# leejaehot/GaussianGrasper

Hardware: AMD Instinct MI355X
Metric: rendered views/sec (fwd+bwd) at 1M Gaussians, 1600x1200, 32-ch feature (higher is better)
Workload: dtype f32; 1 GPU; BASELINE config 4 per-GPU share: 1000000 Gaussians, 1600x1200, SH deg 4 rgb + 32-ch feature + depth + normal images per view (nerfstudio plugin route: the timed callable is FusedGaussianSplattingModel.get_outputs(camera) of gaussiangrasper_amd.plugin (the class train.sh loads, on stub.py's stand-ins for nerfstudio's base model and Cameras) — one fused rasterize operator per view), fwd+bwd, 8 views; route=plugin, deterministic_backward=False, python_gc=gc.freeze() after the warm-up (bench.freeze_gc), view_pipeline=backward of view k beside forward of view k + 1 on two streams, num_gaussians=1000000, feature_dim=32, n_visible=992125, parallelism=view-parallel x1, replicated Gaussians, grad_allreduce_bytes=472000000, grad_allreduce=per parameter, overlapped with the last view's backward

## Files before the change

gaussiangrasper_amd/csrc/binning.hip:

```cpp
#include "scan.h"

__device__ __forceinline__ int64_t dev_count(int64_t n, const int64_t *__restrict__ n_dev) {
    if (n_dev) {
        const int64_t d = *n_dev;
        if (d < n) n = d;
    }
    return n;
}

#define RS_THREADS 256
#define RS_WAVES (RS_THREADS / GG_WAVE)
#ifndef GG_RS_BIG
#define GG_RS_BIG 16
#endif
static inline int rs_items(int64_t n) { return n >= (int64_t)4096 * 1024 ? GG_RS_BIG : 4; }

__global__ __launch_bounds__(256) void count_kernel(int N, const int32_t *__restrict__ nth,
                                                    unsigned long long *__restrict__ out) {
    __shared__ unsigned long long part[4];
    unsigned long long acc = 0;
    for (int i = blockIdx.x * blockDim.x + threadIdx.x; i < N; i += gridDim.x * blockDim.x)
        acc += (unsigned long long)(uint32_t)nth[i];
    for (int off = 32; off > 0; off >>= 1) acc += __shfl_down(acc, off, 64);
    if ((threadIdx.x & 63) == 0) part[threadIdx.x >> 6] = acc;
    __syncthreads();
    if (threadIdx.x == 0) atomicAdd(out, part[0] + part[1] + part[2] + part[3]);
}

extern "C" size_t gg_count_workspace(int num_points) {
    (void)num_points;
    return 0;
}
extern "C" int gg_count_intersects(int N, const int32_t *num_tiles_hit, int64_t *out, void *ws,
                                   size_t ws_bytes, gg_stream_t stream) {
    (void)ws;
    (void)ws_bytes;
    GG_REQUIRE(N >= 0, "num_points < 0");
    GG_REQUIRE(out != nullptr, "null output");
    hipStream_t s = (hipStream_t)stream;
    if (gg_fill_async(out, 0, sizeof(int64_t), s) != hipSuccess) {
        gg_set_error("gg_count_intersects: memset failed");
        return GG_ERR_LAUNCH;
    }
    if (N == 0) return GG_OK;
    GG_REQUIRE(num_tiles_hit != nullptr, "null pointer");
    int blocks = min((N + 255) / 256, 128);
    gg_prof_begin(GG_K_COUNT, s);
    hipLaunchKernelGGL(count_kernel, dim3(blocks), dim3(256), 0, s, N, num_tiles_hit,
                       (unsigned long long *)out);
    gg_prof_end(GG_K_COUNT, s);
    GG_CHECK_LAUNCH();
    return GG_OK;
}

struct DepthSrc {
    const float *depths;
    const int32_t *radii;
};
__device__ __forceinline__ uint32_t depth_key(const DepthSrc d, int64_t idx) {
    return (d.radii[idx] > 0) ? __builtin_bit_cast(uint32_t, d.depths[idx]) : 0xFFFFFFFFu;
}

template <int RS_ITEMS>
__global__ __launch_bounds__(RS_THREADS) void radix_hist_kernel(
    int64_t n, const int64_t *__restrict__ n_dev, const uint32_t *__restrict__ keys, int shift,
    uint32_t mask, int nblocks, uint32_t *__restrict__ G, DepthSrc dsrc) {
    constexpr int RS_TILE = RS_THREADS * RS_ITEMS;
    __shared__ uint32_t hist[256];
    n = dev_count(n, n_dev);
    hist[threadIdx.x] = 0;
    __syncthreads();
    int64_t base = (int64_t)blockIdx.x * RS_TILE;
#pragma unroll 4
    for (int it = 0; it < RS_ITEMS; ++it) {
        int64_t idx = base + (int64_t)it * RS_THREADS + threadIdx.x;
        if (idx < n) atomicAdd(&hist[((dsrc.depths ? depth_key(dsrc, idx) : keys[idx]) >> shift) & mask], 1u);
    }
    __syncthreads();
    G[(size_t)threadIdx.x * nblocks + blockIdx.x] = hist[threadIdx.x];
}

__global__ __launch_bounds__(256) void radix_colscan_kernel(int nblocks, uint32_t *__restrict__ G,
                                                            uint32_t *__restrict__ totals) {
    __shared__ uint32_t wsum[4];
    __shared__ uint32_t carry_s;
    uint32_t *row = G + (size_t)blockIdx.x * nblocks;
    const int lane = threadIdx.x & 63, wave = threadIdx.x >> 6;
    if (threadIdx.x == 0) carry_s = 0;
    __syncthreads();
    for (int start = 0; start < nblocks; start += 256) {
        int i = start + threadIdx.x;
        uint32_t v = (i < nblocks) ? row[i] : 0u;
        uint32_t incl = v;
        for (int off = 1; off < 64; off <<= 1) {
            uint32_t t = __shfl_up(incl, off, 64);
            if (lane >= off) incl += t;
        }
        if (lane == 63) wsum[wave] = incl;
        __syncthreads();
        uint32_t wpre = 0;
        for (int w = 0; w < wave; ++w) wpre += wsum[w];
        uint32_t carry = carry_s;
        if (i < nblocks) row[i] = carry + wpre + incl - v;
        __syncthreads();
        if (threadIdx.x == 255) carry_s = carry + wpre + incl;
        __syncthreads();
    }
    if (threadIdx.x == 0) totals[blockIdx.x] = carry_s;
}

template <int RS_ITEMS>
__global__ __launch_bounds__(RS_THREADS) void radix_scatter_kernel(
    int64_t n, const int64_t *__restrict__ n_dev, const uint32_t *__restrict__ keys_in,
    const uint32_t *__restrict__ vals_in, uint32_t *__restrict__ keys_out,
    uint32_t *__restrict__ vals_out, int shift, uint32_t mask, int nblocks,
    const uint32_t *__restrict__ G, const uint32_t *__restrict__ totals, DepthSrc dsrc) {
    constexpr int RS_TILE = RS_THREADS * RS_ITEMS;
    n = dev_count(n, n_dev);
    const int nbits = 32 - __builtin_clz(mask | 1u);
    __shared__ uint32_t whist[RS_WAVES][256];
    __shared__ uint32_t digit_base[256];
    __shared__ uint32_t wsum[4];
    const int tid = threadIdx.x, lane = tid & 63, wave = tid >> 6;
    {
        uint32_t v = totals[tid];
        uint32_t incl = v;
        for (int off = 1; off < 64; off <<= 1) {
            uint32_t t = __shfl_up(incl, off, 64);
            if (lane >= off) incl += t;
        }
        if (lane == 63) wsum[wave] = incl;
        for (int w = 0; w < RS_WAVES; ++w) whist[w][tid] = 0;
        __syncthreads();
        uint32_t wpre = 0;
        for (int w = 0; w < wave; ++w) wpre += wsum[w];
        digit_base[tid] = wpre + incl - v + G[(size_t)tid * nblocks + blockIdx.x];
    }
    __syncthreads();

    const int64_t wbase = (int64_t)blockIdx.x * RS_TILE + (int64_t)wave * (GG_WAVE * RS_ITEMS);
    uint32_t key[RS_ITEMS], val[RS_ITEMS], rank[RS_ITEMS];
    const uint64_t lt_mask = (lane == 0) ? 0ull : (~0ull >> (64 - lane));
#pragma unroll
    for (int it = 0; it < RS_ITEMS; ++it) {
        int64_t idx = wbase + (int64_t)it * GG_WAVE + lane;
        bool valid = idx < n;
        key[it] = valid ? (dsrc.depths ? depth_key(dsrc, idx) : keys_in[idx]) : 0u;
        val[it] = valid ? (dsrc.depths ? (uint32_t)idx : vals_in[idx]) : 0u;
    }
#pragma unroll
    for (int it = 0; it < RS_ITEMS; ++it) {
        int64_t idx = wbase + (int64_t)it * GG_WAVE + lane;
        bool valid = idx < n;
        uint32_t d = (key[it] >> shift) & mask;
        uint64_t peers = __ballot(valid);
#pragma unroll
        for (int b = 0; b < 8; ++b) {
            if (b < nbits) {
                bool bit = (d >> b) & 1u;
                uint64_t m = __ballot(bit);
                peers &= bit ? m : ~m;
            }
        }
        uint32_t cnt = (uint32_t)__popcll(peers);
        uint32_t before = (uint32_t)__popcll(peers & lt_mask);
        uint32_t old = 0u;
        if (valid && before == 0) old = atomicAdd(&whist[wave][d], cnt);
        old = __shfl(old, (int)__builtin_ctzll(peers | (1ull << 63)), 64);
        rank[it] = old + before;
    }
    __syncthreads();
    __shared__ uint32_t lstart[256];
    __shared__ uint32_t skey[RS_TILE], sval[RS_TILE];
    {
        uint32_t run = 0;
        for (int w = 0; w < RS_WAVES; ++w) {
            uint32_t c = whist[w][tid];
            whist[w][tid] = run;
            run += c;
        }
        uint32_t incl = run;
        for (int off = 1; off < 64; off <<= 1) {
            uint32_t u = __shfl_up(incl, off, 64);
            if (lane >= off) incl += u;
        }
        if (lane == 63) wsum[wave] = incl;
        __syncthreads();
        uint32_t wpre = 0;
        for (int w = 0; w < wave; ++w) wpre += wsum[w];
        lstart[tid] = wpre + incl - run;
    }
    __syncthreads();
#pragma unroll
    for (int it = 0; it < RS_ITEMS; ++it) {
        int64_t idx = wbase + (int64_t)it * GG_WAVE + lane;
        if (idx < n) {
            uint32_t d = (key[it] >> shift) & mask;
            uint32_t lp = lstart[d] + whist[wave][d] + rank[it];
            skey[lp] = key[it];
            sval[lp] = val[it];
        }
    }
    __syncthreads();
    const int64_t left = n - (int64_t)blockIdx.x * RS_TILE;
    const int count = (int)(left < RS_TILE ? left : RS_TILE);
    for (int jj = tid; jj < count; jj += RS_THREADS) {
        const uint32_t k = skey[jj];
        const uint32_t d = (k >> shift) & mask;
        const uint32_t dst = digit_base[d] + ((uint32_t)jj - lstart[d]);
        keys_out[dst] = k;
        vals_out[dst] = sval[jj];
    }
}


typedef unsigned long long u64;
#define DB_BLOCKS 64
#define DB_THREADS 1024
#define DB_CAP 512
// ... 451 lines not shown
#pragma unroll
            for (int r = 0; r < DB_ITEMS; ++r) gid[r] = (c0 + 64 * r + lane < n) ? (uint32_t)pairs[s0 + c0 + 64 * r + lane] : 0u;
        }
#pragma unroll
        for (int r = 0; r < DB_ITEMS; ++r) {
            const int p = c0 + 64 * r + lane;
            if (c0 + 64 * r < n) {
                const bool valid = p < n;
                const uint32_t g = min(gid[r], (uint32_t)(N - 1));
                uint32_t c = cntv[r], bx = boxv[r];
                if (!carried) {
                    c = 0u;
                    bx = 1u << 20;
                    if (valid) db_box(geom, dsrc, (int)g, c, bx);
                }
                if (!valid) c = 0u;
                uint32_t incl = c;
#pragma unroll
                for (int off = 1; off < 64; off <<= 1) {
                    const uint32_t u = __shfl_up(incl, off, 64);
                    if (lane >= off) incl += u;
                }
                if (valid) {
                    order[s0 + p] = g;
                    einfo[s0 + p] = make_uint4(carry + incl - c, (uint32_t)b, bx, c);
                }
                carry += __shfl(incl, 63, 64);
            }
        }
    }
    if (lane == 0) bucket_sum[b] = carry;
}

__global__ __launch_bounds__(256) void emit_kernel(int N, const uint32_t *__restrict__ order,
                                                   const uint4 *__restrict__ einfo,
                                                   const uint32_t *__restrict__ bucket_base,
                                                   const uint32_t *__restrict__ visible, int tiles_x,
                                                   int64_t I, const int64_t *__restrict__ I_dev,
                                                   uint32_t *__restrict__ tkeys,
                                                   uint32_t *__restrict__ tvals) {
    __shared__ uint32_t s_rel[4][64];
    I = dev_count(I, I_dev);
    __shared__ int4 s_box[4][64];
    const int lane = threadIdx.x & 63, wave = threadIdx.x >> 6;
    const int r = blockIdx.x * blockDim.x + threadIdx.x;
    uint32_t g = 0, cnt = 0, off = 0;
    int x0 = 0, y0 = 0, bw = 1;
    if (r < N && (uint32_t)r < *visible) {
        g = min(order[r], (uint32_t)(N - 1));
        const uint4 e = einfo[r];
        off = e.x + bucket_base[e.y];
        x0 = (int)(e.z & 1023u);
        y0 = (int)((e.z >> 10) & 1023u);
        bw = max(1, (int)(e.z >> 20));
        cnt = e.w;
    }
    uint32_t incl = cnt;
    for (int d = 1; d < 64; d <<= 1) {
        uint32_t u = __shfl_up(incl, d, 64);
        if (lane >= d) incl += u;
    }
    const uint32_t total = __shfl(incl, 63, 64);
    const uint32_t base = __shfl(off, 0, 64);
    s_rel[wave][lane] = incl - cnt;
    s_box[wave][lane] = make_int4(x0, y0, bw, (int)g);
    __builtin_amdgcn_wave_barrier();
    const uint32_t *rel = s_rel[wave];
    for (uint32_t j = lane; j < total; j += 64) {
        int lo = 0;
#pragma unroll
        for (int step = 32; step > 0; step >>= 1)
            if (rel[lo + step] <= j) lo += step;
        const int4 b = s_box[wave][lo];
        const uint32_t k = j - rel[lo];
        const uint32_t row = k / (uint32_t)b.z;
        const int64_t cur = (int64_t)base + j;
        if (cur < I) {
            tkeys[cur] = (uint32_t)((b.y + (int)row) * tiles_x + b.x + (int)(k - row * (uint32_t)b.z));
            tvals[cur] = (uint32_t)b.w;
        }
    }
}

__global__ __launch_bounds__(256) void tile_bins_kernel(int64_t I, const int64_t *__restrict__ I_dev,
                                                        const uint32_t *__restrict__ tkeys_sorted,
                                                        uint32_t num_tiles,
                                                        int32_t *__restrict__ tile_bins,
                                                        int32_t *__restrict__ tile_out) {
    I = dev_count(I, I_dev);
    int64_t i = (int64_t)blockIdx.x * blockDim.x + threadIdx.x;
    if (i >= I) return;
    uint32_t cur = tkeys_sorted[i];
    if (tile_out) tile_out[i] = (int32_t)cur;
    const bool cur_ok = cur < num_tiles;
    if (i == 0 && cur_ok) tile_bins[2 * cur] = 0;
    if (i == I - 1 && cur_ok) tile_bins[2 * cur + 1] = (int32_t)I;
    if (i > 0) {
        uint32_t prev = tkeys_sorted[i - 1];
        if (prev != cur) {
            if (prev < num_tiles) tile_bins[2 * prev + 1] = (int32_t)i;
            if (cur_ok) tile_bins[2 * cur] = (int32_t)i;
        }
    }
}

static int radix_nblocks(int64_t n) {
    const int64_t tile = (int64_t)RS_THREADS * rs_items(n);
    return (int)((n + tile - 1) / tile);
}

struct BinWs {
    uint32_t *order;
    uint4 *einfo;
    uint32_t *G;
    uint32_t *totals;
    uint32_t *tkeyA, *tkeyB, *tvalTmp;
    uint4 *recs;
    u64 *pairs;
    uint32_t *dbG;
    uint32_t *dbStart;
    uint32_t *dbBase;
    uint32_t *dbmm;
    size_t bytes;
};
static BinWs bin_ws_layout(void *ws, int N, int64_t I) {
    BinWs w;
    size_t off = 0;
    auto take = [&](size_t nbytes) {
        char *p = ws ? (char *)ws + off : nullptr;
        off += gg_align_up(nbytes, 256);
        return (uint32_t *)p;
    };
    size_t n = (size_t)(N > 0 ? N : 1), i = (size_t)(I > 0 ? I : 1);
    w.order = take(4 * n);
    w.einfo = (uint4 *)take(16 * n);
    int nb = max(radix_nblocks(N), radix_nblocks(I));
    w.G = take(4 * 256 * (size_t)(nb + 1));
    w.totals = take(4 * 256);
    w.tkeyA = take(4 * i);
    w.tkeyB = take(4 * i);
    w.tvalTmp = take(4 * i);
    const size_t nbk = (size_t)db_buckets(N);
    w.recs = (uint4 *)take(16 * n);
    w.pairs = (u64 *)take(8 * n);
    w.dbG = take(4 * DB_BLOCKS * (nbk + 1));
    w.dbStart = take(4 * (nbk + 2));
    w.dbBase = take(4 * (nbk + 1));
    w.dbmm = take(4 * 2 * 256);
    w.bytes = off;
    return w;
}
extern "C" size_t gg_bin_sort_workspace(int num_points, int64_t num_intersects) {
    return bin_ws_layout(nullptr, num_points, num_intersects).bytes;
}

static void radix_pass(int64_t n, const int64_t *n_dev, const uint32_t *kin, const uint32_t *vin,
                       uint32_t *kout, uint32_t *vout, int shift, uint32_t mask, BinWs &w, hipStream_t s,
                       DepthSrc dsrc = DepthSrc{nullptr, nullptr}) {
    int nb = radix_nblocks(n);
    if (rs_items(n) != 4)
        hipLaunchKernelGGL(radix_hist_kernel<GG_RS_BIG>, dim3(nb), dim3(RS_THREADS), 0, s, n, n_dev, kin, shift,
                           mask, nb, w.G, dsrc);
    else
        hipLaunchKernelGGL(radix_hist_kernel<4>, dim3(nb), dim3(RS_THREADS), 0, s, n, n_dev, kin, shift,
                           mask, nb, w.G, dsrc);
    hipLaunchKernelGGL(radix_colscan_kernel, dim3(256), dim3(256), 0, s, nb, w.G, w.totals);
    if (rs_items(n) != 4)
        hipLaunchKernelGGL(radix_scatter_kernel<GG_RS_BIG>, dim3(nb), dim3(RS_THREADS), 0, s, n, n_dev, kin, vin,
                           kout, vout, shift, mask, nb, w.G, w.totals, dsrc);
    else
        hipLaunchKernelGGL(radix_scatter_kernel<4>, dim3(nb), dim3(RS_THREADS), 0, s, n, n_dev, kin, vin,
                           kout, vout, shift, mask, nb, w.G, w.totals, dsrc);
}

static int bin_sort_impl(int N, int64_t I, const int64_t *I_dev, const float *xys, const float *depths,
                         const int32_t *radii, const int32_t *num_tiles_hit, int tiles_x, int tiles_y,
                         int32_t *gaussian_ids_sorted, int32_t *tile_bins, int32_t *isect_tile_sorted,
                         void *ws, size_t ws_bytes, gg_stream_t stream, const uint32_t *range_lo = nullptr,
                         const uint32_t *range_hi = nullptr, int range_parts = 0) {
    GG_REQUIRE(N >= 0 && I >= 0, "negative size");
    GG_REQUIRE(tiles_x > 0 && tiles_y > 0, "empty tile grid");
    GG_REQUIRE(tiles_x <= DB_BOX_MAX && tiles_y <= DB_BOX_MAX, "tile grid beyond 1023 x 1023 (images beyond 16 368 pixels a side)");
    GG_REQUIRE(I < (int64_t)1 << 31, "num_intersects must fit int32 (tile_bins are int32)");
    GG_REQUIRE(tile_bins != nullptr, "null tile_bins");
    hipStream_t s = (hipStream_t)stream;
    const int T = tiles_x * tiles_y;
    if (N == 0 || I == 0) {
        if (gg_fill_async(tile_bins, 0, sizeof(int32_t) * 2 * (size_t)T, s) != hipSuccess) {
            gg_set_error("gg_bin_sort: memset failed");
            return GG_ERR_LAUNCH;
        }
        return GG_OK;
    }
    GG_REQUIRE(xys && depths && radii && num_tiles_hit && gaussian_ids_sorted, "null pointer");
    BinWs w = bin_ws_layout(ws, N, I);
    if (ws == nullptr || ws_bytes < w.bytes) {
        gg_set_error("gg_bin_sort: workspace too small (%zu < %zu)", ws_bytes, w.bytes);
        return GG_ERR_WORKSPACE;
    }
    gg_prof_begin(GG_K_BIN_SORT, s);
    const int nbk = db_buckets(N);
    const DepthSrc dsrc{depths, radii};
    const size_t walk_lds = sizeof(uint32_t) * ((size_t)nbk + 1 + 2);
    if (walk_lds > 64 * 1024) {
        (void)hipFuncSetAttribute((const void *)db_walk_kernel<false>, hipFuncAttributeMaxDynamicSharedMemorySize, (int)walk_lds);
        (void)hipFuncSetAttribute((const void *)db_walk_kernel<true>, hipFuncAttributeMaxDynamicSharedMemorySize, (int)walk_lds);
    }
    uint32_t *order = w.order;
    DbParts mm{w.dbmm, w.dbmm + 256, 256};
    if (range_lo && range_hi && range_parts > 0)
        mm = DbParts{range_lo, range_hi, range_parts};
    else
        hipLaunchKernelGGL(db_range_kernel, dim3(256), dim3(256), 0, s, N, dsrc, w.dbmm);
    const DbGeom geom{xys, tiles_x, tiles_y};
    hipLaunchKernelGGL(db_walk_kernel<false>, dim3(DB_BLOCKS), dim3(DB_THREADS), walk_lds, s, N, nbk, dsrc, geom, mm,
                       w.dbG, (const uint32_t *)nullptr, (uint4 *)nullptr, tile_bins, 2 * T);
    hipLaunchKernelGGL(db_prefix_kernel, dim3((nbk + 1 + 255) / 256), dim3(256), 0, s, nbk, w.dbG, w.dbStart);
    hipLaunchKernelGGL(db_scan_kernel, dim3(1), dim3(1024), 0, s, nbk, w.dbStart);
    hipLaunchKernelGGL(db_walk_kernel<true>, dim3(DB_BLOCKS), dim3(DB_THREADS), walk_lds, s, N, nbk, dsrc, geom, mm,
                       w.dbG, (const uint32_t *)w.dbStart, w.recs, (int32_t *)nullptr, 0);
    hipLaunchKernelGGL(db_sort_kernel, dim3((nbk + DB_WPB - 1) / DB_WPB), dim3(64 * DB_WPB), 0, s, N, nbk,
                       (const uint32_t *)w.dbStart, (const uint4 *)w.recs, w.pairs, dsrc, geom, order, w.einfo, w.dbBase);
    hipLaunchKernelGGL(db_scan_kernel, dim3(1), dim3(1024), 0, s, nbk, w.dbBase);
    int tile_bits = 1;
    while ((1 << tile_bits) < T) ++tile_bits;
    int passes = (tile_bits + 7) / 8;
    uint32_t *out_vals = (uint32_t *)gaussian_ids_sorted;
    uint32_t *kcur = w.tkeyA, *kalt = w.tkeyB;
    uint32_t *vcur = (passes % 2 == 0) ? out_vals : w.tvalTmp;
    uint32_t *valt = (passes % 2 == 0) ? w.tvalTmp : out_vals;
    if (!I_dev) {
        (void)gg_fill_async(kcur, 0xFF, sizeof(uint32_t) * (size_t)I, s);
        (void)gg_fill_async(vcur, 0, sizeof(uint32_t) * (size_t)I, s);
    }
    hipLaunchKernelGGL(emit_kernel, dim3((N + 255) / 256), dim3(256), 0, s, N, (const uint32_t *)order,
                       (const uint4 *)w.einfo, (const uint32_t *)w.dbBase, (const uint32_t *)(w.dbStart + nbk), tiles_x, I,
                       I_dev, kcur, vcur);
    const int per_pass = (tile_bits + passes - 1) / passes;
    for (int pass = 0; pass < passes; ++pass) {
        int bits = min(per_pass, tile_bits - per_pass * pass);
        radix_pass(I, I_dev, kcur, vcur, kalt, valt, per_pass * pass, (1u << bits) - 1u, w, s);
        uint32_t *t = kcur; kcur = kalt; kalt = t;
        t = vcur; vcur = valt; valt = t;
    }
    hipLaunchKernelGGL(tile_bins_kernel, dim3((unsigned)((I + 255) / 256)), dim3(256), 0, s, I, I_dev, kcur,
                       (uint32_t)T, tile_bins, isect_tile_sorted);
    gg_prof_end(GG_K_BIN_SORT, s);
    GG_CHECK_LAUNCH();
    return GG_OK;
}

extern "C" int gg_bin_sort_status(int N, int64_t I, const void *ws, size_t ws_bytes, gg_stream_t stream) {
    GG_REQUIRE(N >= 0 && I >= 0, "negative size");
    (void)ws;
    (void)ws_bytes;
    if (hipStreamSynchronize((hipStream_t)stream) != hipSuccess) {
        gg_set_error("gg_bin_sort_status: stream synchronisation failed");
        return GG_ERR_LAUNCH;
    }
    return GG_OK;
}

extern "C" int gg_bin_sort(int N, int64_t I, const float *xys, const float *depths,
                           const int32_t *radii, const int32_t *num_tiles_hit, int tiles_x,
                           int tiles_y, int32_t *gaussian_ids_sorted, int32_t *tile_bins,
                           int32_t *isect_tile_sorted, void *ws, size_t ws_bytes,
                           gg_stream_t stream) {
    return bin_sort_impl(N, I, nullptr, xys, depths, radii, num_tiles_hit, tiles_x, tiles_y,
                         gaussian_ids_sorted, tile_bins, isect_tile_sorted, ws, ws_bytes, stream);
}

extern "C" int gg_bin_sort_dev(int N, int64_t capacity, const int64_t *num_intersects_dev,
                               const float *xys, const float *depths, const int32_t *radii,
                               const int32_t *num_tiles_hit, int tiles_x, int tiles_y,
                               int32_t *gaussian_ids_sorted, int32_t *tile_bins,
                               int32_t *isect_tile_sorted, void *ws, size_t ws_bytes,
                               gg_stream_t stream) {
    GG_REQUIRE(num_intersects_dev != nullptr, "null num_intersects_dev");
    GG_REQUIRE(capacity >= 1, "capacity < 1");
    return bin_sort_impl(N, capacity, num_intersects_dev, xys, depths, radii, num_tiles_hit, tiles_x,
                         tiles_y, gaussian_ids_sorted, tile_bins, isect_tile_sorted, ws, ws_bytes, stream);
}

extern "C" int gg_bin_sort_dev_ex(int N, int64_t capacity, const int64_t *num_intersects_dev,
                                  const float *xys, const float *depths, const int32_t *radii,
                                  const int32_t *num_tiles_hit, int tiles_x, int tiles_y,
                                  int32_t *gaussian_ids_sorted, int32_t *tile_bins,
                                  int32_t *isect_tile_sorted, void *ws, size_t ws_bytes,
                                  const uint32_t *depth_bits_min, const uint32_t *depth_bits_max, int range_parts,
                                  gg_stream_t stream) {
    GG_REQUIRE(num_intersects_dev != nullptr, "null num_intersects_dev");
    GG_REQUIRE(capacity >= 1, "capacity < 1");
    GG_REQUIRE(range_parts == 0 || (depth_bits_min && depth_bits_max && range_parts > 0), "range parts without arrays");
    return bin_sort_impl(N, capacity, num_intersects_dev, xys, depths, radii, num_tiles_hit, tiles_x,
                         tiles_y, gaussian_ids_sorted, tile_bins, isect_tile_sorted, ws, ws_bytes, stream,
                         depth_bits_min, depth_bits_max, range_parts);
}

size_t gg_sort_pairs_workspace(int64_t n) {
    const size_t i = (size_t)(n > 0 ? n : 1);
    return gg_align_up(4 * i, 256) * 2 + gg_align_up(4 * 256 * (size_t)(radix_nblocks(n) + 1), 256) +
           gg_align_up(4 * 256, 256);
}
int gg_sort_pairs(int64_t n, uint32_t *keys, uint32_t *vals, int bits, void *ws, size_t ws_bytes, hipStream_t s) {
    if (n <= 0) return GG_OK;
    if (ws == nullptr || ws_bytes < gg_sort_pairs_workspace(n)) return GG_ERR_WORKSPACE;
    char *p = (char *)ws;
    const size_t i = (size_t)n;
    uint32_t *kalt = (uint32_t *)p;
    p += gg_align_up(4 * i, 256);
    uint32_t *valt = (uint32_t *)p;
    p += gg_align_up(4 * i, 256);
    BinWs w;
    w.G = (uint32_t *)p;
    p += gg_align_up(4 * 256 * (size_t)(radix_nblocks(n) + 1), 256);
    w.totals = (uint32_t *)p;
    uint32_t *kc = keys, *vc = vals, *ka = kalt, *va = valt;
    const int passes = (bits + 7) / 8;
    for (int pass = 0; pass < passes; ++pass) {
        const int b = min(8, bits - 8 * pass);
        radix_pass(n, nullptr, kc, vc, ka, va, 8 * pass, (1u << b) - 1u, w, s);
        uint32_t *t = kc; kc = ka; ka = t;
        t = vc; vc = va; va = t;
    }
    if (kc != keys) {
        if (hipMemcpyAsync(keys, kc, 4 * i, hipMemcpyDeviceToDevice, s) != hipSuccess) return GG_ERR_LAUNCH;
        if (hipMemcpyAsync(vals, vc, 4 * i, hipMemcpyDeviceToDevice, s) != hipSuccess) return GG_ERR_LAUNCH;
    }
// ... 3 lines not shown
```

gaussiangrasper_amd/csrc/gg_common.h:

```cpp
#pragma once
#include <hip/hip_runtime.h>
#include <stdint.h>

#include "../../include/gg_constants.h"
#include "../../include/gg_raster.h"

#define GG_WAVE 64

void gg_set_error(const char *fmt, ...);

#define GG_REQUIRE(cond, msg)                      \
    do {                                           \
        if (!(cond)) {                             \
            gg_set_error("%s: %s", __func__, msg); \
            return GG_ERR_INVALID_ARG;             \
        }                                          \
    } while (0)

#define GG_CHECK_LAUNCH()                                                   \
    do {                                                                    \
        hipError_t e__ = hipGetLastError();                                 \
        if (e__ != hipSuccess) {                                            \
            gg_set_error("%s: launch failed: %s", __func__, hipGetErrorString(e__)); \
            return GG_ERR_LAUNCH;                                           \
        }                                                                   \
    } while (0)

void gg_prof_begin(int kernel_id, hipStream_t s);
void gg_prof_end(int kernel_id, hipStream_t s);
static inline int gg_width_index(int w) {
    return w <= 1 ? 0 : w <= 3 ? 1 : w == 4 ? 2 : w == 8 ? 3 : w == 16 ? 4 : 5;
}

static inline size_t gg_align_up(size_t x, size_t a) { return (x + a - 1) / a * a; }

struct GgCarve {
    char *base;
    size_t off;
    char *take(size_t bytes) {
        char *p = base ? base + off : nullptr;
        off += gg_align_up(bytes, 256);
        return p;
    }
};

#define GG_REQUIRE_WS(ws, ws_bytes, need)                                                              \
    do {                                                                                               \
        GG_REQUIRE((ws) && ((uintptr_t)(ws) & 255) == 0, "ws must be non-null and 256-byte aligned");  \
        if ((ws_bytes) < (need)) {                                                                     \
            gg_set_error("%s: workspace too small: %zu < %zu bytes", __func__, (size_t)(ws_bytes),     \
                         (size_t)(need));                                                              \
            return GG_ERR_WORKSPACE;                                                                   \
        }                                                                                              \
    } while (0)

static __global__ __launch_bounds__(256) void gg_fill_kernel(uint32_t *__restrict__ p, uint32_t v, size_t nwords,
                                                             int vec) {
    const size_t i = ((size_t)blockIdx.x * 256 + threadIdx.x) * 4;
    if (vec && i + 3 < nwords) {
        *reinterpret_cast<uint4 *>(p + i) = make_uint4(v, v, v, v);
    } else {
        for (int k = 0; k < 4; ++k)
            if (i + k < nwords) p[i + k] = v;
    }
}
static inline hipError_t gg_fill_async(void *p, int byte, size_t bytes, hipStream_t s) {
    if (bytes == 0) return hipSuccess;
    if ((reinterpret_cast<uintptr_t>(p) & 3) || (bytes & 3)) return hipMemsetAsync(p, byte, bytes, s);
    uint32_t v = (uint32_t)byte & 0xffu;
    v |= v << 8;
    v |= v << 16;
    const size_t nwords = bytes / 4;
    const unsigned blocks = (unsigned)((nwords + 1023) / 1024);
    hipLaunchKernelGGL(gg_fill_kernel, dim3(blocks), dim3(256), 0, s, reinterpret_cast<uint32_t *>(p), v, nwords,
                       (reinterpret_cast<uintptr_t>(p) & 15) == 0 ? 1 : 0);
    return hipGetLastError();
}

__device__ __forceinline__ float gg_expf(float x) {
    float t = x * GG_EXP_LOG2E;
    float n = __builtin_rintf(t);
    float r = __builtin_fmaf(n, -GG_EXP_LN2_HI, x);
    r = __builtin_fmaf(n, -GG_EXP_LN2_LO, r);
    float p = GG_EXP_P0;
    p = __builtin_fmaf(p, r, GG_EXP_P1);
    p = __builtin_fmaf(p, r, GG_EXP_P2);
    p = __builtin_fmaf(p, r, GG_EXP_P3);
    p = __builtin_fmaf(p, r, GG_EXP_P4);
    p = __builtin_fmaf(p, r, GG_EXP_P5);
    float z = r * r;
    float y = __builtin_fmaf(p, z, r);
    y = y + 1.0f;
    float s = __builtin_bit_cast(float, (uint32_t)((int)n + 127) << 23);
    float e = y * s;
    return (x < GG_EXP_LO) ? 0.0f : e;
}

__device__ __forceinline__ float gg_expf_walk(float x) {
#ifdef GG_EXP_PROBE
    return __builtin_amdgcn_exp2f(x * GG_EXP_LOG2E);
#endif
    float t = x * GG_EXP_LOG2E;
    float n = __builtin_rintf(t);
    float r = __builtin_fmaf(n, -GG_EXP_LN2_HI, x);
    r = __builtin_fmaf(n, -GG_EXP_LN2_LO, r);
    float p = GG_EXP_P0;
    p = __builtin_fmaf(p, r, GG_EXP_P1);
    p = __builtin_fmaf(p, r, GG_EXP_P2);
    p = __builtin_fmaf(p, r, GG_EXP_P3);
    p = __builtin_fmaf(p, r, GG_EXP_P4);
    p = __builtin_fmaf(p, r, GG_EXP_P5);
    float z = r * r;
    float y = __builtin_fmaf(p, z, r);
    y = y + 1.0f;
    return __builtin_amdgcn_ldexpf(y, (int)n);
}

typedef float f32x2 __attribute__((ext_vector_type(2)));
typedef _Float16 h16x2 __attribute__((ext_vector_type(2)));
typedef _Float16 h16x8 __attribute__((ext_vector_type(8)));
typedef unsigned u32x4 __attribute__((ext_vector_type(4)));
__device__ __forceinline__ void split2h(float x0, float x1, unsigned &hi, unsigned &lo) {
    const h16x2 h = __builtin_convertvector((f32x2){x0, x1}, h16x2);
    const f32x2 back = __builtin_convertvector(h, f32x2);
    const h16x2 l = __builtin_convertvector((f32x2){x0 - back[0], x1 - back[1]}, h16x2);
    hi = __builtin_bit_cast(unsigned, h);
    lo = __builtin_bit_cast(unsigned, l);
}
__device__ __forceinline__ float pow2_scale(float m) {
    const unsigned e = (__builtin_bit_cast(unsigned, m) >> 23) & 0xffu;
    return __builtin_bit_cast(float, min(268u - e, 253u) << 23);
}
__device__ __forceinline__ float pow2_inv(float s) {
    return __builtin_bit_cast(float, (254u << 23) - __builtin_bit_cast(unsigned, s));
}
#define H8(a, b, c, d) __builtin_bit_cast(h16x8, (u32x4){(a), (b), (c), (d)})

// ... 13 lines not shown
```

gaussiangrasper_amd/csrc/project.hip:

```cpp
#include <stdarg.h>
#include <stdio.h>

#include "blend_common.h"

static thread_local char g_err[512] = "";
void gg_set_error(const char *fmt, ...) {
    va_list ap;
    va_start(ap, fmt);
    vsnprintf(g_err, sizeof(g_err), fmt, ap);
    va_end(ap);
}
extern "C" const char *gg_last_error(void) { return g_err; }
extern "C" int gg_abi_version(void) { return 6; }

__device__ __forceinline__ void quat_to_R(const float4 q, float *R, float *qn, float &inv) {
    float nn = ((q.x * q.x + q.y * q.y) + q.z * q.z) + q.w * q.w;
    inv = 1.0f / sqrtf(nn);
    float w = q.x * inv, x = q.y * inv, y = q.z * inv, z = q.w * inv;
    R[0] = 1.0f - 2.0f * (y * y + z * z);
    R[1] = 2.0f * (x * y - w * z);
    R[2] = 2.0f * (x * z + w * y);
    R[3] = 2.0f * (x * y + w * z);
    R[4] = 1.0f - 2.0f * (x * x + z * z);
    R[5] = 2.0f * (y * z - w * x);
// ... 709 lines not shown
                              gg_stream_t stream) {
    return gg_project_bwd_ex(N, means3d, scales, glob_scale, quats, viewmat, projmat, fx, fy, cx, cy, img_height,
                             img_width, radii, conics, v_xy, 2, v_depth, v_conic, 3, v_mean3d, 0, v_scale, v_quat,
                             stream);
}
extern "C" int gg_project_bwd_ex(int N, const float *means3d, const float *scales, float glob_scale,
                                 const float *quats, const float *viewmat, const float *projmat,
                                 float fx, float fy, float cx, float cy, int img_height,
                                 int img_width, const int32_t *radii, const float *conics,
                                 const float *v_xy, int v_xy_stride, const float *v_depth, const float *v_conic,
                                 int v_conic_stride, float *v_mean3d, int accumulate_means, float *v_scale,
                                 float *v_quat, gg_stream_t stream) {
    (void)cx;
    (void)cy;
    GG_REQUIRE(v_xy_stride >= 2 && v_conic_stride >= 3, "v_xy rows hold 2 values, v_conic rows 3");
    GG_REQUIRE(N >= 0, "num_points < 0");
    if (N == 0) return GG_OK;
    GG_REQUIRE(means3d && scales && quats && viewmat && projmat && radii && conics && v_xy &&
                   v_depth && v_conic && v_mean3d && v_scale && v_quat,
               "null pointer");
    gg_prof_begin(GG_K_PROJECT_BWD, (hipStream_t)stream);
    hipLaunchKernelGGL(project_bwd_kernel, dim3((N + 255) / 256), dim3(256), 0,
                       (hipStream_t)stream, N, means3d, scales, glob_scale, quats, viewmat,
                       projmat, fx, fy, img_height, img_width, radii, conics, v_xy, v_depth,
                       v_conic, v_mean3d, v_scale, v_quat, v_xy_stride, v_conic_stride, accumulate_means);
    gg_prof_end(GG_K_PROJECT_BWD, (hipStream_t)stream);
    GG_CHECK_LAUNCH();
    return GG_OK;
}

template <int K>
static void launch_sh(bool fwd, bool acc, int N, int deg, const float *viewdirs, const float *in, float *out,
                      hipStream_t s) {
    dim3 grid((N + 255) / 256), block(256);
    const int rows_fwd = 4 * ((K >= 16) ? 32 : 64);
    if (fwd)
        hipLaunchKernelGGL(sh_fwd_kernel<K>, dim3((N + rows_fwd - 1) / rows_fwd), block, 0, s, N, deg,
                           viewdirs, in, out);
    else if (acc)
        hipLaunchKernelGGL((sh_bwd_kernel<K, true>), grid, block, 0, s, N, deg, viewdirs, in, out);
    else
        hipLaunchKernelGGL((sh_bwd_kernel<K, false>), grid, block, 0, s, N, deg, viewdirs, in, out);
}

static int sh_dispatch(bool fwd, bool acc, int N, int K, int deg, const float *viewdirs, const float *in,
                       float *out, gg_stream_t stream) {
    GG_REQUIRE(N >= 0, "num_points < 0");
    GG_REQUIRE(K == 1 || K == 4 || K == 9 || K == 16 || K == 25, "num_bases must be 1,4,9,16,25");
    GG_REQUIRE(deg >= 0 && sh_nbases(deg) <= K, "degrees_to_use exceeds stored bases");
    if (N == 0) return GG_OK;
    GG_REQUIRE(viewdirs && in && out, "null pointer");
    hipStream_t s = (hipStream_t)stream;
    gg_prof_begin(fwd ? GG_K_SH_FWD : GG_K_SH_BWD, s);
    switch (K) {
        case 1: launch_sh<1>(fwd, acc, N, deg, viewdirs, in, out, s); break;
        case 4: launch_sh<4>(fwd, acc, N, deg, viewdirs, in, out, s); break;
        case 9: launch_sh<9>(fwd, acc, N, deg, viewdirs, in, out, s); break;
        case 16: launch_sh<16>(fwd, acc, N, deg, viewdirs, in, out, s); break;
        default: launch_sh<25>(fwd, acc, N, deg, viewdirs, in, out, s); break;
    }
    gg_prof_end(fwd ? GG_K_SH_FWD : GG_K_SH_BWD, s);
    GG_CHECK_LAUNCH();
    return GG_OK;
}
extern "C" int gg_sh_fwd(int N, int K, int deg, const float *viewdirs, const float *coeffs,
                         float *colors, gg_stream_t stream) {
    return sh_dispatch(true, false, N, K, deg, viewdirs, coeffs, colors, stream);
}
extern "C" int gg_sh_bwd(int N, int K, int deg, const float *viewdirs, const float *v_colors,
                         float *v_coeffs, gg_stream_t stream) {
    return sh_dispatch(false, false, N, K, deg, viewdirs, v_colors, v_coeffs, stream);
}
extern "C" int gg_sh_bwd_accumulate(int N, int K, int deg, const float *viewdirs, const float *v_colors,
                                    float *v_coeffs, gg_stream_t stream) {
    return sh_dispatch(false, true, N, K, deg, viewdirs, v_colors, v_coeffs, stream);
}

#define GG_SH_MULTI_VIEWS 16
struct ShMultiArgs {
    const float *viewdirs[GG_SH_MULTI_VIEWS];
    const float *v_colors[GG_SH_MULTI_VIEWS];
    int num_views;
};
template <int K, bool ACC>
__global__ __launch_bounds__(256) void sh_bwd_multi_kernel(int N, int deg, ShMultiArgs a,
                                                           float *__restrict__ v_coeffs) {
    constexpr int ROW = 3 * K;
    __shared__ float stage[4][64 * ROW];
    const int lane = threadIdx.x & 63, wave = threadIdx.x >> 6;
    const int base = (blockIdx.x * 4 + wave) * 64;
    if (base >= N) return;
    const int nrows = min(64, N - base);
    float *st = stage[wave];
    const int i = base + lane;
    float *dst = v_coeffs + (size_t)base * ROW;
    if (ACC) {
        for (int e = lane; e < nrows * ROW; e += 64) st[e] = dst[e];
        __builtin_amdgcn_wave_barrier();
    }
    if (lane < nrows) {
        float acc[ROW];
        float *row0 = st + lane * ROW;
#pragma unroll
        for (int e = 0; e < ROW; ++e) acc[e] = ACC ? row0[e] : 0.0f;
        const int nb = min(sh_nbases(deg), K);
        for (int v = 0; v < a.num_views; ++v) {
            const float *vd = a.viewdirs[v] + 3 * (size_t)i;
            const float *vc = a.v_colors[v] + 3 * (size_t)i;
            float Y[GG_SH_MAX_BASES];
            sh_basis(deg, vd[0], vd[1], vd[2], Y);
            const float c0 = vc[0], c1 = vc[1], c2 = vc[2];
#pragma unroll
            for (int k = 0; k < K; ++k)
                if (k < nb) {
                    acc[3 * k + 0] = acc[3 * k + 0] + Y[k] * c0;
                    acc[3 * k + 1] = acc[3 * k + 1] + Y[k] * c1;
                    acc[3 * k + 2] = acc[3 * k + 2] + Y[k] * c2;
                }
        }
        float *row = st + lane * ROW;
#pragma unroll
        for (int e = 0; e < ROW; ++e) row[e] = acc[e];
    }
    __builtin_amdgcn_wave_barrier();
    for (int e = lane; e < nrows * ROW; e += 64) dst[e] = st[e];
}
__global__ __launch_bounds__(256) void tail_split_kernel(int N, const float *__restrict__ v_tail, int vstride,
                                                         const uint8_t *__restrict__ mask,
                                                         float *__restrict__ v_rgb, float *__restrict__ v_depths,
                                                         float *__restrict__ v_normals) {
    const int i = blockIdx.x * blockDim.x + threadIdx.x;
    if (i >= N) return;
    const float *vt = v_tail + (size_t)i * vstride;
    const unsigned m = mask[i];
#pragma unroll
    for (int c = 0; c < 3; ++c) v_rgb[3 * (size_t)i + c] = ((m >> c) & 1u) ? vt[c] : 0.0f;
    v_depths[i] = vt[3];
#pragma unroll
    for (int c = 0; c < 3; ++c) v_normals[3 * (size_t)i + c] = vt[4 + c];
}
extern "C" int gg_shade_tail_bwd_split(int N, const float *v_tail, int v_tail_stride, const uint8_t *clamp_mask,
                                       float *v_rgb, float *v_depths, float *v_normals, gg_stream_t stream) {
    GG_REQUIRE(N >= 0, "num_points < 0");
    GG_REQUIRE(v_tail_stride >= 7, "v_tail rows hold 7 values");
    if (N == 0) return GG_OK;
    GG_REQUIRE(v_tail && clamp_mask && v_rgb && v_depths && v_normals, "null pointer");
    gg_prof_begin(GG_K_TAIL_SPLIT, (hipStream_t)stream);
    hipLaunchKernelGGL(tail_split_kernel, dim3((N + 255) / 256), dim3(256), 0, (hipStream_t)stream, N, v_tail,
                       v_tail_stride, clamp_mask, v_rgb, v_depths, v_normals);
    gg_prof_end(GG_K_TAIL_SPLIT, (hipStream_t)stream);
    GG_CHECK_LAUNCH();
    return GG_OK;
}
template <int K>
static void launch_sh_multi(bool acc, int N, int deg, const ShMultiArgs &a, float *out, hipStream_t s) {
    dim3 grid((N + 255) / 256), block(256);
    if (acc) hipLaunchKernelGGL((sh_bwd_multi_kernel<K, true>), grid, block, 0, s, N, deg, a, out);
    else hipLaunchKernelGGL((sh_bwd_multi_kernel<K, false>), grid, block, 0, s, N, deg, a, out);
}
extern "C" int gg_sh_bwd_multi(int N, int K, int deg, int num_views, const float *const *viewdirs,
                               const float *const *v_colors, float *v_coeffs, int accumulate, gg_stream_t stream) {
    GG_REQUIRE(N >= 0, "num_points < 0");
    GG_REQUIRE(K == 1 || K == 4 || K == 9 || K == 16 || K == 25, "num_bases must be 1,4,9,16,25");
    GG_REQUIRE(deg >= 0 && sh_nbases(deg) <= K, "degrees_to_use exceeds stored bases");
    GG_REQUIRE(num_views >= 1, "num_views < 1");
    if (N == 0) return GG_OK;
    GG_REQUIRE(viewdirs && v_colors && v_coeffs, "null pointer");
    hipStream_t s = (hipStream_t)stream;
    gg_prof_begin(GG_K_SH_BWD, s);
    for (int first = 0; first < num_views; first += GG_SH_MULTI_VIEWS) {
        ShMultiArgs a;
        a.num_views = min(GG_SH_MULTI_VIEWS, num_views - first);
        for (int v = 0; v < GG_SH_MULTI_VIEWS; ++v) {
            const int src = first + (v < a.num_views ? v : 0);
            GG_REQUIRE(viewdirs[src] && v_colors[src], "null view pointer");
            a.viewdirs[v] = viewdirs[src];
            a.v_colors[v] = v_colors[src];
        }
        const bool acc = accumulate != 0 || first > 0;
        switch (K) {
            case 1: launch_sh_multi<1>(acc, N, deg, a, v_coeffs, s); break;
            case 4: launch_sh_multi<4>(acc, N, deg, a, v_coeffs, s); break;
            case 9: launch_sh_multi<9>(acc, N, deg, a, v_coeffs, s); break;
            case 16: launch_sh_multi<16>(acc, N, deg, a, v_coeffs, s); break;
            default: launch_sh_multi<25>(acc, N, deg, a, v_coeffs, s); break;
        }
    }
    gg_prof_end(GG_K_SH_BWD, s);
    GG_CHECK_LAUNCH();
    return GG_OK;
}

template <int K>
static void launch_tail(bool fwd, bool acc, int N, int deg, const float *viewdirs, const float *in, float *out,
                        const float *depths, const float *normals, uint8_t *mask, int vstride, float *v_depths,
                        float *v_normals, hipStream_t s, bool one_wave = false) {
    dim3 grid((N + 255) / 256), block(256);
    const int rows_fwd = 4 * ((K >= 16) ? 32 : 64);
    if (fwd && one_wave)
        hipLaunchKernelGGL((sh_fwd_kernel<K, true, 1>), dim3((N + rows_fwd / 4 - 1) / (rows_fwd / 4)), dim3(64), 0, s, N,
                           deg, viewdirs, in, out, depths, normals, mask);
    else if (fwd)
        hipLaunchKernelGGL((sh_fwd_kernel<K, true>), dim3((N + rows_fwd - 1) / rows_fwd), block, 0, s, N, deg,
                           viewdirs, in, out, depths, normals, mask);
    else if (acc)
        hipLaunchKernelGGL((sh_bwd_kernel<K, true, true>), grid, block, 0, s, N, deg, viewdirs, in, out, vstride,
                           mask, v_depths, v_normals);
    else
// ... 555 lines not shown
```

Before: 650.3 views/s.

## Vectorize radix histogram and tile-bin loads, halve SH backward staging LDS

Radix histogram reads sort keys as 16-byte vectors when aligned, and the colscan and digit work is limited to live digits (mask+1 blocks). tile_bins becomes a grid-stride kernel that handles four keys per thread with vector loads and stores, getting the previous key through a shuffle. The SH multi-view backward kernel stages its rows in two 32-row halves to cut shared memory and raise occupancy, copies with float4, prefetches the next view's inputs and sets min-blocks launch bounds. These reduce memory instruction count and LDS pressure, at the cost of more complex boundary handling.

Result: no change. 648.7 views/s (-0.3%).

```diff
diff --git a/gaussiangrasper_amd/csrc/binning.hip b/gaussiangrasper_amd/csrc/binning.hip
--- a/gaussiangrasper_amd/csrc/binning.hip
+++ b/gaussiangrasper_amd/csrc/binning.hip
@@ -71,13 +71,38 @@
     hist[threadIdx.x] = 0;
     __syncthreads();
     int64_t base = (int64_t)blockIdx.x * RS_TILE;
+    if (!dsrc.depths && (reinterpret_cast<uintptr_t>(keys) & 15) == 0) {
+        static_assert(RS_ITEMS % 4 == 0, "keys per thread: a multiple of four");
+        uint4 q[RS_ITEMS / 4];
+#pragma unroll
+        for (int it = 0; it < RS_ITEMS / 4; ++it) {
+            const int64_t idx = base + ((int64_t)it * RS_THREADS + threadIdx.x) * 4;
+            if (idx + 4 <= n) {
+                q[it] = *reinterpret_cast<const uint4 *>(keys + idx);
+            } else {
+                q[it].x = idx < n ? keys[idx] : 0u;
+                q[it].y = idx + 1 < n ? keys[idx + 1] : 0u;
+                q[it].z = idx + 2 < n ? keys[idx + 2] : 0u;
+                q[it].w = 0u;
+            }
+        }
+#pragma unroll
+        for (int it = 0; it < RS_ITEMS / 4; ++it) {
+            const int64_t idx = base + ((int64_t)it * RS_THREADS + threadIdx.x) * 4;
+            if (idx < n) atomicAdd(&hist[(q[it].x >> shift) & mask], 1u);
+            if (idx + 1 < n) atomicAdd(&hist[(q[it].y >> shift) & mask], 1u);
+            if (idx + 2 < n) atomicAdd(&hist[(q[it].z >> shift) & mask], 1u);
+            if (idx + 3 < n) atomicAdd(&hist[(q[it].w >> shift) & mask], 1u);
+        }
+    } else {
 #pragma unroll 4
-    for (int it = 0; it < RS_ITEMS; ++it) {
-        int64_t idx = base + (int64_t)it * RS_THREADS + threadIdx.x;
-        if (idx < n) atomicAdd(&hist[((dsrc.depths ? depth_key(dsrc, idx) : keys[idx]) >> shift) & mask], 1u);
+        for (int it = 0; it < RS_ITEMS; ++it) {
+            int64_t idx = base + (int64_t)it * RS_THREADS + threadIdx.x;
+            if (idx < n) atomicAdd(&hist[((dsrc.depths ? depth_key(dsrc, idx) : keys[idx]) >> shift) & mask], 1u);
+        }
     }
     __syncthreads();
-    G[(size_t)threadIdx.x * nblocks + blockIdx.x] = hist[threadIdx.x];
+    if (threadIdx.x <= mask) G[(size_t)threadIdx.x * nblocks + blockIdx.x] = hist[threadIdx.x];
 }
 
 __global__ __launch_bounds__(256) void radix_colscan_kernel(int nblocks, uint32_t *__restrict__ G,
@@ -123,7 +148,8 @@
     __shared__ uint32_t wsum[4];
     const int tid = threadIdx.x, lane = tid & 63, wave = tid >> 6;
     {
-        uint32_t v = totals[tid];
+        const bool live = (uint32_t)tid <= mask;
+        uint32_t v = live ? totals[tid] : 0u;
         uint32_t incl = v;
         for (int off = 1; off < 64; off <<= 1) {
             uint32_t t = __shfl_up(incl, off, 64);
@@ -134,7 +160,7 @@
         __syncthreads();
         uint32_t wpre = 0;
         for (int w = 0; w < wave; ++w) wpre += wsum[w];
-        digit_base[tid] = wpre + incl - v + G[(size_t)tid * nblocks + blockIdx.x];
+        digit_base[tid] = live ? wpre + incl - v + G[(size_t)tid * nblocks + blockIdx.x] : 0u;
     }
     __syncthreads();
 
@@ -752,24 +778,54 @@
     }
 }
 
+#define TB_KEYS 4
+#define TB_CHUNK (256 * TB_KEYS)
+#define TB_WGS_PER_CU 8
 __global__ __launch_bounds__(256) void tile_bins_kernel(int64_t I, const int64_t *__restrict__ I_dev,
                                                         const uint32_t *__restrict__ tkeys_sorted,
                                                         uint32_t num_tiles,
                                                         int32_t *__restrict__ tile_bins,
                                                         int32_t *__restrict__ tile_out) {
     I = dev_count(I, I_dev);
-    int64_t i = (int64_t)blockIdx.x * blockDim.x + threadIdx.x;
-    if (i >= I) return;
-    uint32_t cur = tkeys_sorted[i];
-    if (tile_out) tile_out[i] = (int32_t)cur;
-    const bool cur_ok = cur < num_tiles;
-    if (i == 0 && cur_ok) tile_bins[2 * cur] = 0;
-    if (i == I - 1 && cur_ok) tile_bins[2 * cur + 1] = (int32_t)I;
-    if (i > 0) {
-        uint32_t prev = tkeys_sorted[i - 1];
-        if (prev != cur) {
-            if (prev < num_tiles) tile_bins[2 * prev + 1] = (int32_t)i;
-            if (cur_ok) tile_bins[2 * cur] = (int32_t)i;
+    const bool wide_in = (reinterpret_cast<uintptr_t>(tkeys_sorted) & 15) == 0;
+    const bool wide_out = tile_out && (reinterpret_cast<uintptr_t>(tile_out) & 15) == 0;
+    const int lane = threadIdx.x & 63;
+    for (int64_t c = (int64_t)blockIdx.x * TB_CHUNK; c < I; c += (int64_t)gridDim.x * TB_CHUNK) {
+        const int64_t i0 = c + (int64_t)threadIdx.x * TB_KEYS;
+        const bool whole = i0 + TB_KEYS <= I;
+        uint32_t k[TB_KEYS];
+        if (whole && wide_in) {
+            const uint4 q = *reinterpret_cast<const uint4 *>(tkeys_sorted + i0);
+            k[0] = q.x; k[1] = q.y; k[2] = q.z; k[3] = q.w;
+        } else {
+#pragma unroll
+            for (int j = 0; j < TB_KEYS; ++j) k[j] = i0 + j < I ? tkeys_sorted[i0 + j] : 0u;
+        }
+        uint32_t prev = __shfl_up(k[TB_KEYS - 1], 1, 64);
+        if (lane == 0 && i0 > 0 && i0 < I) prev = tkeys_sorted[i0 - 1];
+        if (tile_out) {
+            if (whole && wide_out) {
+                *reinterpret_cast<int4 *>(tile_out + i0) = make_int4((int)k[0], (int)k[1], (int)k[2], (int)k[3]);
+            } else {
+#pragma unroll
+                for (int j = 0; j < TB_KEYS; ++j)
+                    if (i0 + j < I) tile_out[i0 + j] = (int32_t)k[j];
+            }
+        }
+#pragma unroll
+        for (int j = 0; j < TB_KEYS; ++j) {
+            const int64_t i = i0 + j;
+            const uint32_t cur = k[j];
+            if (i < I) {
+                const bool cur_ok = cur < num_tiles;
+                if (i == 0 && cur_ok) tile_bins[2 * cur] = 0;
+                if (i == I - 1 && cur_ok) tile_bins[2 * cur + 1] = (int32_t)I;
+                if (i > 0 && prev != cur) {
+                    if (prev < num_tiles) tile_bins[2 * prev + 1] = (int32_t)i;
+                    if (cur_ok) tile_bins[2 * cur] = (int32_t)i;
+                }
+            }
+            prev = cur;
         }
     }
 }
@@ -824,23 +880,23 @@
     return bin_ws_layout(nullptr, num_points, num_intersects).bytes;
 }
 
+template <int ITEMS>
+static void radix_launch(int nb, int64_t n, const int64_t *n_dev, const uint32_t *kin, const uint32_t *vin, uint32_t *kout,
+                         uint32_t *vout, int shift, uint32_t mask, BinWs &w, hipStream_t s, DepthSrc dsrc) {
+    hipLaunchKernelGGL(radix_hist_kernel<ITEMS>, dim3(nb), dim3(RS_THREADS), 0, s, n, n_dev, kin, shift, mask, nb, w.G,
+                       dsrc);
+    hipLaunchKernelGGL(radix_colscan_kernel, dim3(mask + 1), dim3(256), 0, s, nb, w.G, w.totals);
+    hipLaunchKernelGGL(radix_scatter_kernel<ITEMS>, dim3(nb), dim3(RS_THREADS), 0, s, n, n_dev, kin, vin, kout, vout,
+                       shift, mask, nb, w.G, w.totals, dsrc);
+}
 static void radix_pass(int64_t n, const int64_t *n_dev, const uint32_t *kin, const uint32_t *vin,
                        uint32_t *kout, uint32_t *vout, int shift, uint32_t mask, BinWs &w, hipStream_t s,
                        DepthSrc dsrc = DepthSrc{nullptr, nullptr}) {
     int nb = radix_nblocks(n);
-    if (rs_items(n) != 4)
-        hipLaunchKernelGGL(radix_hist_kernel<GG_RS_BIG>, dim3(nb), dim3(RS_THREADS), 0, s, n, n_dev, kin, shift,
-                           mask, nb, w.G, dsrc);
-    else
-        hipLaunchKernelGGL(radix_hist_kernel<4>, dim3(nb), dim3(RS_THREADS), 0, s, n, n_dev, kin, shift,
-                           mask, nb, w.G, dsrc);
-    hipLaunchKernelGGL(radix_colscan_kernel, dim3(256), dim3(256), 0, s, nb, w.G, w.totals);
-    if (rs_items(n) != 4)
-        hipLaunchKernelGGL(radix_scatter_kernel<GG_RS_BIG>, dim3(nb), dim3(RS_THREADS), 0, s, n, n_dev, kin, vin,
-                           kout, vout, shift, mask, nb, w.G, w.totals, dsrc);
-    else
-        hipLaunchKernelGGL(radix_scatter_kernel<4>, dim3(nb), dim3(RS_THREADS), 0, s, n, n_dev, kin, vin,
-                           kout, vout, shift, mask, nb, w.G, w.totals, dsrc);
+    switch (rs_items(n)) {
+        case 4: radix_launch<4>(nb, n, n_dev, kin, vin, kout, vout, shift, mask, w, s, dsrc); break;
+        default: radix_launch<GG_RS_BIG>(nb, n, n_dev, kin, vin, kout, vout, shift, mask, w, s, dsrc); break;
+    }
 }
 
 static int bin_sort_impl(int N, int64_t I, const int64_t *I_dev, const float *xys, const float *depths,
@@ -913,7 +969,8 @@
         uint32_t *t = kcur; kcur = kalt; kalt = t;
         t = vcur; vcur = valt; valt = t;
     }
-    hipLaunchKernelGGL(tile_bins_kernel, dim3((unsigned)((I + 255) / 256)), dim3(256), 0, s, I, I_dev, kcur,
+    hipLaunchKernelGGL(tile_bins_kernel, dim3(gg_stride_grid((size_t)((I + TB_CHUNK - 1) / TB_CHUNK), TB_WGS_PER_CU)),
+                       dim3(256), 0, s, I, I_dev, kcur,
                        (uint32_t)T, tile_bins, isect_tile_sorted);
     gg_prof_end(GG_K_BIN_SORT, s);
     GG_CHECK_LAUNCH();
diff --git a/gaussiangrasper_amd/csrc/gg_common.h b/gaussiangrasper_amd/csrc/gg_common.h
--- a/gaussiangrasper_amd/csrc/gg_common.h
+++ b/gaussiangrasper_amd/csrc/gg_common.h
@@ -53,6 +53,23 @@
             return GG_ERR_WORKSPACE;                                                                   \
         }                                                                                              \
     } while (0)
+
+static inline int gg_cu_count() {
+    static const int cus = [] {
+        int dev = 0, v = 0;
+        if (hipGetDevice(&dev) != hipSuccess ||
+            hipDeviceGetAttribute(&v, hipDeviceAttributeMultiprocessorCount, dev) != hipSuccess || v <= 0)
+            v = 256;
+        return v;
+    }();
+    return cus;
+}
+static inline unsigned gg_stride_grid(size_t chunks, int wgs_per_cu) {
+    const size_t cap = (size_t)wgs_per_cu * (size_t)gg_cu_count();
+    if (chunks <= cap) return (unsigned)(chunks < 1 ? 1 : chunks);
+    const size_t iters = (chunks + cap - 1) / cap;
+    return (unsigned)((chunks + iters - 1) / iters);
+}
 
 static __global__ __launch_bounds__(256) void gg_fill_kernel(uint32_t *__restrict__ p, uint32_t v, size_t nwords,
                                                              int vec) {
diff --git a/gaussiangrasper_amd/csrc/project.hip b/gaussiangrasper_amd/csrc/project.hip
--- a/gaussiangrasper_amd/csrc/project.hip
+++ b/gaussiangrasper_amd/csrc/project.hip
@@ -815,11 +815,31 @@
     const float *v_colors[GG_SH_MULTI_VIEWS];
     int num_views;
 };
+#define SHM_ROWS 32
+template <bool TO_STAGE>
+__device__ __forceinline__ void shm_copy(float *__restrict__ st, float *__restrict__ g, int count, bool wide, int lane) {
+    int done = 0;
+    if (wide) {
+        const int n4 = count >> 2;
+        float4 *s4 = reinterpret_cast<float4 *>(st);
+        float4 *g4 = reinterpret_cast<float4 *>(g);
+#pragma unroll 4
+        for (int e = lane; e < n4; e += 64) {
+            if (TO_STAGE) s4[e] = g4[e];
+            else g4[e] = s4[e];
+        }
+        done = n4 << 2;
+    }
+    for (int e = done + lane; e < count; e += 64) {
+        if (TO_STAGE) st[e] = g[e];
+        else g[e] = st[e];
+    }
+}
 template <int K, bool ACC>
-__global__ __launch_bounds__(256) void sh_bwd_multi_kernel(int N, int deg, ShMultiArgs a,
+__global__ __launch_bounds__(256, ACC ? 4 : 3) void sh_bwd_multi_kernel(int N, int deg, ShMultiArgs a,
                                                            float *__restrict__ v_coeffs) {
     constexpr int ROW = 3 * K;
-    __shared__ float stage[4][64 * ROW];
+    __shared__ __attribute__((aligned(16))) float stage[4][SHM_ROWS * ROW];
     const int lane = threadIdx.x & 63, wave = threadIdx.x >> 6;
     const int base = (blockIdx.x * 4 + wave) * 64;
     if (base >= N) return;
@@ -827,36 +847,68 @@
     float *st = stage[wave];
     const int i = base + lane;
     float *dst = v_coeffs + (size_t)base * ROW;
+    const bool wide = (reinterpret_cast<uintptr_t>(v_coeffs) & 15) == 0;
+    const bool mine = lane < nrows;
+    float *row = st + (lane & (SHM_ROWS - 1)) * ROW;
+    float d0 = 0.0f, d1 = 0.0f, d2 = 0.0f, c0 = 0.0f, c1 = 0.0f, c2 = 0.0f;
+    if (mine) {
+        const float *vd = a.viewdirs[0] + 3 * (size_t)i;
+        const float *vc = a.v_colors[0] + 3 * (size_t)i;
+        d0 = vd[0]; d1 = vd[1]; d2 = vd[2];
+        c0 = vc[0]; c1 = vc[1]; c2 = vc[2];
+    }
+    float acc[ROW];
+#pragma unroll
+    for (int e = 0; e < ROW; ++e) acc[e] = 0.0f;
     if (ACC) {
-        for (int e = lane; e < nrows * ROW; e += 64) st[e] = dst[e];
-        __builtin_amdgcn_wave_barrier();
-    }
-    if (lane < nrows) {
-        float acc[ROW];
-        float *row0 = st + lane * ROW;
-#pragma unroll
-        for (int e = 0; e < ROW; ++e) acc[e] = ACC ? row0[e] : 0.0f;
+#pragma unroll
+        for (int half = 0; half < 64 / SHM_ROWS; ++half) {
+            const int r0 = half * SHM_ROWS;
+            if (r0 < nrows) {
+                shm_copy<true>(st, dst + (size_t)r0 * ROW, (min(nrows, r0 + SHM_ROWS) - r0) * ROW, wide, lane);
+                __builtin_amdgcn_wave_barrier();
+                if (mine && (lane / SHM_ROWS) == half) {
+#pragma unroll
+                    for (int e = 0; e < ROW; ++e) acc[e] = row[e];
+                }
+                __builtin_amdgcn_wave_barrier();
+            }
+        }
+    }
+    if (mine) {
         const int nb = min(sh_nbases(deg), K);
         for (int v = 0; v < a.num_views; ++v) {
-            const float *vd = a.viewdirs[v] + 3 * (size_t)i;
-            const float *vc = a.v_colors[v] + 3 * (size_t)i;
+            const float x = d0, y = d1, z = d2, g0 = c0, g1 = c1, g2 = c2;
+            if (v + 1 < a.num_views) {
+                const float *vd = a.viewdirs[v + 1] + 3 * (size_t)i;
+                const float *vc = a.v_colors[v + 1] + 3 * (size_t)i;
+                d0 = vd[0]; d1 = vd[1]; d2 = vd[2];
+                c0 = vc[0]; c1 = vc[1]; c2 = vc[2];
+            }
             float Y[GG_SH_MAX_BASES];
-            sh_basis(deg, vd[0], vd[1], vd[2], Y);
-            const float c0 = vc[0], c1 = vc[1], c2 = vc[2];
+            sh_basis(deg, x, y, z, Y);
 #pragma unroll
             for (int k = 0; k < K; ++k)
                 if (k < nb) {
-                    acc[3 * k + 0] = acc[3 * k + 0] + Y[k] * c0;
-                    acc[3 * k + 1] = acc[3 * k + 1] + Y[k] * c1;
-                    acc[3 * k + 2] = acc[3 * k + 2] + Y[k] * c2;
+                    acc[3 * k + 0] = acc[3 * k + 0] + Y[k] * g0;
+                    acc[3 * k + 1] = acc[3 * k + 1] + Y[k] * g1;
+                    acc[3 * k + 2] = acc[3 * k + 2] + Y[k] * g2;
                 }
         }
-        float *row = st + lane * ROW;
-#pragma unroll
-        for (int e = 0; e < ROW; ++e) row[e] = acc[e];
-    }
-    __builtin_amdgcn_wave_barrier();
-    for (int e = lane; e < nrows * ROW; e += 64) dst[e] = st[e];
+    }
+#pragma unroll
+    for (int half = 0; half < 64 / SHM_ROWS; ++half) {
+        const int r0 = half * SHM_ROWS;
+        if (r0 < nrows) {
+            if (mine && (lane / SHM_ROWS) == half) {
+#pragma unroll
+                for (int e = 0; e < ROW; ++e) row[e] = acc[e];
+            }
+            __builtin_amdgcn_wave_barrier();
+            shm_copy<false>(st, dst + (size_t)r0 * ROW, (min(nrows, r0 + SHM_ROWS) - r0) * ROW, wide, lane);
+            __builtin_amdgcn_wave_barrier();
+        }
+    }
 }
 __global__ __launch_bounds__(256) void tail_split_kernel(int N, const float *__restrict__ v_tail, int vstride,
                                                          const uint8_t *__restrict__ mask,
```
